# caizexin/GenVC

Hardware: AMD Instinct MI355X
Metric: utterances/s (streaming, 1 s chunks; with RTF and first-chunk latency) (higher is better)
Workload: dtype f32; 1 GPU; GenVC_small streaming, 1 s chunks, top_k=1, batch 1 per GPU (BASELINE configs[1]); parallelism=replicas x1, utterances sharded by rank, all_gather of token ids

## Files before the change

### genvc_amd/csrc/gemm.h

```cpp
#pragma once
#include "common.h"

namespace gvc {

__host__ __device__ __forceinline__ size_t fm16_index(int m, int k, int K) {
    return ((size_t)(m >> 4) * (K >> 4) + (k >> 4)) * 256 + (size_t)((((m & 15) + 16 * ((k & 15) >> 2)) << 2) + (k & 3));
}

enum GemmAct { ACT_NONE = 0, ACT_GELU_NEW = 1, ACT_RELU = 2, ACT_GELU_ERF = 3 };
enum GemmAAct { AACT_NONE = 0, AACT_LRELU = 1 };

struct GemmEpi {
    const float* bias;
    long long bias_batch_stride;
    int act;
    const float* resid;
    int ldr;
    long long resid_batch_stride;
    long long resid_batch_stride2;
    int resid_fm16;
    int geglu;
    const float* resid2;
    float out_scale;
    int c_fm16;
// ... 159 lines not shown
        } else {
            const int b = m / e.T, t = m - b * e.T;
            const int h = c / e.head_dim, j = c - h * e.head_dim;
            float* cache = which == 1 ? e.kcache : e.vcache;
            const size_t at = (((size_t)p.slot * e.n_head + h) * e.max_seq + (t + p.base)) * e.head_dim + j;
            if (e.kv_bf16) {
                ushort4 o;
                o.x = f32_to_bf16(v.x); o.y = f32_to_bf16(v.y); o.z = f32_to_bf16(v.z); o.w = f32_to_bf16(v.w);
                *reinterpret_cast<ushort4*>(reinterpret_cast<unsigned short*>(cache) + at) = o;
            } else {
                *reinterpret_cast<float4*>(cache + at) = v;
            }
        }
        return;
    }
    if (e.geglu) {
        *reinterpret_cast<float2*>(G.C + fm16_index(m, n >> 1, G.N >> 1)) = make_float2(gelu_erf(v.y) * v.x, gelu_erf(v.w) * v.z);
        return;
    }
    if (e.resid) {
        const float4 r = *reinterpret_cast<const float4*>(e.resid + (e.resid_fm16 ? fm16_index(m, n, G.N) : (size_t)m * e.ldr + n));
        v.x += r.x; v.y += r.y; v.z += r.z; v.w += r.w;
    }
    if (e.resid2) {
        const float4 r = *reinterpret_cast<const float4*>(e.resid2 + (size_t)m * e.ldr + n);
        v.x += r.x; v.y += r.y; v.z += r.z; v.w += r.w;
    }
    if (e.out_scale != 0.f) { v.x *= e.out_scale; v.y *= e.out_scale; v.z *= e.out_scale; v.w *= e.out_scale; }
    if (e.c_fm16) { *reinterpret_cast<float4*>(G.C + fm16_index(m, n, G.N)) = v; return; }
    *reinterpret_cast<float4*>(G.C + (size_t)m * G.ldc + n) = v;
}

typedef float f32x16 __attribute__((ext_vector_type(16)));

__global__ __launch_bounds__(256) void k_gemm_f32(const GemmArgs G);
__global__ void k_splitk_epilogue(const GemmArgs G);

int launch_gemm_skinny(GemmArgs G, int SK, long long work_cap, hipStream_t s);
int launch_ln_sum_rows(const float* x_in, float* x_out, float* a, const float* part, int SK, const float* bias, int rows, int d,
                       const float* ln_w, const float* ln_b, int a_fm16, hipStream_t s);
struct LnFuse {
    const float* x_in; float* x_out;
    const float* part; int SK; const float* pbias;
    const float* ln_w; const float* ln_b;
    int rows;
};
int launch_gemm_skinny_ln(GemmArgs G, const LnFuse& P, hipStream_t s);
int launch_gemm_strip(GemmArgs G, int sk_max, long long work_cap, int raw_partials, int* sk_used, hipStream_t s);
void gemm_init_attributes();
__global__ void k_to_fm16(const float* src, float* dst, int N, int K);
__global__ void k_to_fm16_bf16(const float* src, unsigned short* dst, int N, int K);

int launch_gemm_cap(GemmArgs G, int batch, long long work_cap, hipStream_t s);

}
```

### genvc_amd/csrc/gemm.hip

```cpp
#include "gemm.h"
#include "gemm_b16.h"
#include <algorithm>

namespace gvc {

constexpr int BM = 64, BN = 64, BK = 32, LDL = 36;

__global__ __launch_bounds__(256) void k_gemm_f32(const GemmArgs G) {
    __shared__ __attribute__((aligned(16))) float As[2][BM * LDL];
    __shared__ __attribute__((aligned(16))) float Bs[2][BN * LDL];
    const int tid = threadIdx.x, lane = tid & 63, wave = tid >> 6;
    const int wm = wave >> 1, wn = wave & 1;
    const int batch = blockIdx.z / G.SK, sk = blockIdx.z - batch * G.SK;
    const int m0 = blockIdx.y * BM, n0 = blockIdx.x * BN;
    const int ntile_all = (G.K + BK - 1) / BK;
    const int tps = (ntile_all + G.SK - 1) / G.SK;
    const int kbeg = sk * tps * BK;
    const int kend = min(G.K, kbeg + tps * BK);
    const int nt = kend > kbeg ? (kend - kbeg + BK - 1) / BK : 0;
    const float* Ab = G.A + gemm_boff(G, batch, G.a_batch_stride, G.a_batch_stride2);
    const float* Wb = G.Wt + gemm_binner(G, batch) * G.w_batch_stride;

    float4 ra[2], rb[2];
    auto load_tile = [&](int kt) {
// ... 34 lines not shown
    if (nt > 0) {
        load_tile(0);
        store_tile(0);
    }
    __syncthreads();
    int buf = 0;
    const int arow = (wm * 32 + (lane & 31)) * LDL + (lane >> 5) * 4;
    const int brow = (wn * 32 + (lane & 31)) * LDL + (lane >> 5) * 4;
    for (int kt = 0; kt < nt; ++kt) {
        if (kt + 1 < nt) load_tile(kt + 1);
#pragma unroll
        for (int kk = 0; kk < 4; ++kk) {
            const float4 a4 = *reinterpret_cast<const float4*>(&As[buf][arow + kk * 8]);
            const float4 b4 = *reinterpret_cast<const float4*>(&Bs[buf][brow + kk * 8]);
            acc = __builtin_amdgcn_mfma_f32_32x32x2f32(a4.x, b4.x, acc, 0, 0, 0);
            acc = __builtin_amdgcn_mfma_f32_32x32x2f32(a4.y, b4.y, acc, 0, 0, 0);
            acc = __builtin_amdgcn_mfma_f32_32x32x2f32(a4.z, b4.z, acc, 0, 0, 0);
            acc = __builtin_amdgcn_mfma_f32_32x32x2f32(a4.w, b4.w, acc, 0, 0, 0);
        }
        if (kt + 1 < nt) store_tile(buf ^ 1);
        __syncthreads();
        buf ^= 1;
    }

    const int n = n0 + wn * 32 + (lane & 31);
#pragma unroll
    for (int r = 0; r < 16; ++r) {
        const int m = m0 + wm * 32 + (r & 3) + 8 * (r >> 2) + 4 * (lane >> 5);
        if (m < G.M && n < G.N) {
            if (G.SK > 1)
                G.work[(((size_t)batch * G.SK + sk) * G.M + m) * G.N + n] = acc[r];
            else
                gemm_store(G, batch, m, n, acc[r]);
        }
    }
}

__global__ void k_splitk_epilogue(const GemmArgs G) {
    const int batch = blockIdx.z;
    const size_t mn = (size_t)G.M * G.N;
    for (size_t i = (size_t)blockIdx.x * blockDim.x + threadIdx.x; i < mn; i += (size_t)gridDim.x * blockDim.x) {
        const float* w = G.work + (size_t)batch * G.SK * mn + i;
        float pv[16];
#pragma unroll
        for (int s = 0; s < 16; ++s) pv[s] = w[(size_t)min(s, G.SK - 1) * mn];
        float v = 0.f;
#pragma unroll
        for (int s = 0; s < 16; ++s)
            if (s < G.SK) v += pv[s];
        gemm_store(G, batch, (int)(i / G.N), (int)(i % G.N), v);
    }
}

int launch_gemm_cap(GemmArgs G, int batch, long long work_cap, hipStream_t s) {
    GVC_REQUIRE(G.K % 4 == 0 && G.lda % 4 == 0 && G.ldw % 4 == 0 && G.conv_cin % 4 == 0 && G.conv_tap_stride % 4 == 0,
                GVC_ERR_ARG, "gemm: K/lda/ldw/conv strides must be multiples of 4 (K=%d lda=%d ldw=%d)", G.K, G.lda, G.ldw);
    const int tm = cdiv(G.M, BM), tn = cdiv(G.N, BN);
    const long long tiles = (long long)tm * tn * batch;
    int SK = 1;
    constexpr int sk_tiles = 128, sk_target = 192;
    if (tiles < sk_tiles && G.work) {
        SK = (int)((sk_target + tiles - 1) / tiles);
        const int max_by_k = G.K / (4 * BK) > 0 ? G.K / (4 * BK) : 1;
        if (SK > max_by_k) SK = max_by_k;
        if (SK > 16) SK = 16;
        while (SK > 1 && (long long)batch * SK * G.M * G.N > work_cap) --SK;
    } else if (tiles < 2 * sk_tiles && G.K >= 64 * BK && G.work) {
        SK = (int)((4 * sk_tiles + tiles - 1) / tiles);
        if (SK > G.K / (16 * BK)) SK = G.K / (16 * BK);
        while (SK > 1 && (long long)batch * SK * G.M * G.N > work_cap) --SK;
    }
    G.SK = SK;
    dim3 grid(tn, tm, batch * SK);
    hipLaunchKernelGGL(k_gemm_f32, grid, dim3(256), 0, s, G);
    GVC_LAUNCH_CHECK();
    if (SK > 1) {
        const long long mn = (long long)G.M * G.N;
        int gx = (int)((mn + 255) / 256);
        if (gx > 2048) gx = 2048;
        hipLaunchKernelGGL(k_splitk_epilogue, dim3(gx, 1, batch), dim3(256), 0, s, G);
        GVC_LAUNCH_CHECK();
    }
    return GVC_OK;
}

typedef float f32x4 __attribute__((ext_vector_type(4)));

template <int WB> struct WRaw { typedef float4 T; };
template <> struct WRaw<1> { typedef uint2 T; };
__device__ __forceinline__ float4 w_f4(const float4& r) { return r; }
__device__ __forceinline__ float4 w_f4(const uint2& u) {
    return make_float4(__uint_as_float(u.x << 16), __uint_as_float(u.x & 0xffff0000u), __uint_as_float(u.y << 16),
                       __uint_as_float(u.y & 0xffff0000u));
}

template <int MT, int NW, int WB = 0, int NC = 0>
__global__ __launch_bounds__(NW * 64) void k_gemm_skinny(const GemmArgs G) {
    extern __shared__ __attribute__((aligned(16))) float red_raw[];
    float (*red)[MT][256] = reinterpret_cast<float (*)[MT][256]>(red_raw);
    const int tid = threadIdx.x, lane = tid & 63, wave = tid >> 6;
    const int r = lane & 15, g = lane >> 4;
    const int n0 = blockIdx.x * 16;
    const int kslice = G.K / G.SK;
    const int kw = kslice / NW;
    const int kb16 = (blockIdx.y * kslice + wave * kw) >> 4;
    const int K16 = G.K >> 4;
    typedef typename WRaw<WB>::T wraw_t;
    const wraw_t* wp = reinterpret_cast<const wraw_t*>(G.Wt) + ((size_t)(n0 >> 4) * K16 + kb16) * 64 + lane;
    const float* ap[MT];
#pragma unroll
    for (int t = 0; t < MT; ++t) ap[t] = G.A + ((size_t)t * K16 + kb16) * 256 + lane * 4;
    f32x4 acc[MT];
#pragma unroll
    for (int t = 0; t < MT; ++t) acc[t] = {0.f, 0.f, 0.f, 0.f};
    EpiPre pre;
    {
        int pm, pn;
        bool four = false;
        if constexpr (MT <= 2) {
            pm = 16 * (tid >> 8) + 4 * (lane >> 4) + ((tid >> 6) & 3); pn = n0 + (lane & 15);
        } else {
            const bool pfm = G.SK == 1 && G.e.c_fm16;
            const int pt = tid >> 6, pj = tid & 63;
            pm = 16 * pt + (pfm ? (pj & 15) : (pj >> 2)); pn = n0 + 4 * (pfm ? (pj >> 4) : (pj & 3));
            four = true;
        }
        if (G.SK == 1) pre = gemm_prefetch(G, min(pm, G.M - 1), pn, four);
    }
    constexpr int U = NC > 0 ? (32 / (MT * NC) >= 8 ? 8 : 32 / (MT * NC)) : (32 / (1 + MT) >= 8 ? 8 : (32 / (1 + MT) >= 4 ? 4 : 2));
    float wn[MT][NC > 0 ? NC : 1], mc[MT][NC > 0 ? NC : 1], lc[MT][NC > 0 ? NC : 1];
    const float* pp[MT];
    if constexpr (NC > 0) {
        const int kg = blockIdx.y * kslice + wave * kw;
        const int h = kg / G.att_hd, pstride = G.att_hd + 4;
#pragma unroll
// ... 739 lines not shown
```

### genvc_amd/csrc/hubert.hip

```cpp
#include <map>
#include <string>
#include <vector>

#include "conv_lds.h"
#include "attn64.h"
#include <algorithm>

namespace gvc {

constexpr int kC0Chunk = 32;

static __global__ void k_hb_repack_conv(const float* w, float* out, int Co, int Ci, int k) {
    const size_t n = (size_t)Co * Ci * k;
    for (size_t i = (size_t)blockIdx.x * blockDim.x + threadIdx.x; i < n; i += (size_t)gridDim.x * blockDim.x) {
        const int j = (int)(i % k);
        const int ci = (int)((i / k) % Ci);
        const int co = (int)(i / ((size_t)k * Ci));
        out[((size_t)co * k + j) * Ci + ci] = w[i];
    }
}

static __global__ __launch_bounds__(256) void k_hb_conv0(const float* wav, const float* w, float* y, float* part, int T,
                                                        int T0, int C, int k, int stride) {
    extern __shared__ float xs[];
    const int b = blockIdx.z, chunk = blockIdx.x, tid = threadIdx.x;
    const int t0 = chunk * kC0Chunk;
    const int nt = min(kC0Chunk, T0 - t0);
    const int nx = (nt - 1) * stride + k;
    const float* src = wav + (size_t)b * T + (size_t)t0 * stride;
    for (int i = tid; i < nx; i += 256) xs[i] = src[i];
    __syncthreads();
    for (int c = blockIdx.y * 256 + tid; c < min(C, (int)(blockIdx.y + 1) * 256); c += 256) {
        float wr[16];
#pragma unroll
        for (int j = 0; j < 16; ++j) wr[j] = j < k ? w[(size_t)c * k + j] : 0.f;
        float s = 0.f, ss = 0.f, a = 0.f;
        float* yo = y + ((size_t)b * T0 + t0) * C + c;
        for (int t = 0; t < nt; ++t) {
            float acc = 0.f;
#pragma unroll
            for (int j = 0; j < 16; ++j)
                if (j < k) acc = fmaf(wr[j], xs[t * stride + j], acc);
            yo[(size_t)t * C] = acc;
            if (t == 0) a = acc;
            const float dv = acc - a;
            s += dv; ss = fmaf(dv, dv, ss);
        }
        float* po = part + (((size_t)b * gridDim.x + chunk) * C + c) * 2;
        const float dm = s / (float)nt;
        po[0] = a + dm; po[1] = fmaxf(ss - s * dm, 0.f);
    }
}

static __global__ __launch_bounds__(256) void k_hb_gn_stats(const float* part, float* stats, int nchunk, int T0, int C) {
    const int b = blockIdx.y, c = blockIdx.x * 8 + (threadIdx.x >> 5), l = threadIdx.x & 31;
    if (c >= C) return;
    double s = 0.0, ss = 0.0;
    for (int i0 = l; i0 < nchunk; i0 += 32 * 8) {
        float2 pv[8];
#pragma unroll
        for (int u = 0; u < 8; ++u)
            pv[u] = *reinterpret_cast<const float2*>(part + (((size_t)b * nchunk + min(i0 + 32 * u, nchunk - 1)) * C + c) * 2);
#pragma unroll
        for (int u = 0; u < 8; ++u)
            if (i0 + 32 * u < nchunk) {
                const double n = (double)min(kC0Chunk, T0 - (i0 + 32 * u) * kC0Chunk), m = (double)pv[u].x;
                s += n * m; ss += (double)pv[u].y + n * m * m;
            }
    }
#pragma unroll
    for (int o = 16; o >= 1; o >>= 1) { s += __shfl_xor(s, o, 32); ss += __shfl_xor(ss, o, 32); }
    if (l) return;
    const double mean = s / T0;
    double var = ss / T0 - mean * mean;
    if (var < 0.0) var = 0.0;
    stats[((size_t)b * C + c) * 2] = (float)mean;
    stats[((size_t)b * C + c) * 2 + 1] = (float)(1.0 / sqrt(var + 1e-5));
}
// ... 19 lines not shown
                                                          const float* part = nullptr, int SK = 0, const float* pbias = nullptr,
                                                          int rows = 0, float* dst_fm16 = nullptr) {
    __shared__ float red[4];
    const int row = blockIdx.x, tid = threadIdx.x;
    const int bi = row / rpb, ri = row - bi * rpb;
    const float* xr = src + bi * src_bs + (size_t)ri * d;
    float* orow = dst + bi * dst_bs + (size_t)ri * d;
    float4 v[4];
    float s = 0.f;
#pragma unroll
    for (int i = 0; i < 4; ++i) {
        const int k = (i * 256 + tid) * 4;
        v[i] = k < d ? *reinterpret_cast<const float4*>(xr + k) : make_float4(0.f, 0.f, 0.f, 0.f);
        if (part && k < d) {
            const float4 b4 = *reinterpret_cast<const float4*>(pbias + k);
            float4 p4[8];
#pragma unroll
            for (int sidx = 0; sidx < 8; ++sidx)
                p4[sidx] = *reinterpret_cast<const float4*>(part + ((size_t)min(sidx, SK - 1) * rows + row) * d + k);
            v[i].x += b4.x; v[i].y += b4.y; v[i].z += b4.z; v[i].w += b4.w;
#pragma unroll
            for (int sidx = 0; sidx < 8; ++sidx)
                if (sidx < SK) { v[i].x += p4[sidx].x; v[i].y += p4[sidx].y; v[i].z += p4[sidx].z; v[i].w += p4[sidx].w; }
        }
        s += (v[i].x + v[i].y) + (v[i].z + v[i].w);
    }
    const float inv_d = 1.0f / (float)d;
    const float mean = block4_sum(s, red) * inv_d;
    float q = 0.f;
#pragma unroll
    for (int i = 0; i < 4; ++i) {
        const int k = (i * 256 + tid) * 4;
        if (k < d) {
            const float a0 = v[i].x - mean, a1 = v[i].y - mean, a2 = v[i].z - mean, a3 = v[i].w - mean;
            q += (a0 * a0 + a1 * a1) + (a2 * a2 + a3 * a3);
        }
    }
    const float rstd = 1.0f / sqrtf(block4_sum(q, red) * inv_d + 1e-5f);
#pragma unroll
    for (int i = 0; i < 4; ++i) {
        const int k = (i * 256 + tid) * 4;
        if (k < d) {
            const float4 gw = *reinterpret_cast<const float4*>(w + k);
            const float4 gb = *reinterpret_cast<const float4*>(b + k);
            float4 o;
            o.x = (v[i].x - mean) * rstd * gw.x + gb.x; o.y = (v[i].y - mean) * rstd * gw.y + gb.y;
            o.z = (v[i].z - mean) * rstd * gw.z + gb.z; o.w = (v[i].w - mean) * rstd * gw.w + gb.w;
            *reinterpret_cast<float4*>(orow + k) = o;
            if (dst_fm16) *reinterpret_cast<float4*>(dst_fm16 + fm16_index(row, k, d)) = o;
        }
    }
}

static __global__ void k_hb_zero_pad(float* buf, int C, int T, int front, int back, const int32_t* fmask) {
    const int b = blockIdx.y;
    float* base = buf + (size_t)b * (front + T + back) * C;
    const size_t nf = (size_t)front * C, nb = (size_t)back * C;
    for (size_t i = (size_t)blockIdx.x * blockDim.x + threadIdx.x; i < nf + nb; i += (size_t)gridDim.x * blockDim.x) {
        if (i < nf) base[i] = 0.f;
        else base[(size_t)(front + T) * C + (i - nf)] = 0.f;
    }
    for (int t = blockIdx.x; t < T; t += gridDim.x) {
        if (!fmask[b * T + t]) continue;
        for (int i = threadIdx.x; i < C; i += blockDim.x) base[(size_t)(front + t) * C + i] = 0.f;
    }
}

static __global__ __launch_bounds__(64) void k_hb_frame_mask(const float* wav, int32_t* fmask, int T, int F) {
    const int f = blockIdx.x, b = blockIdx.y, lane = threadIdx.x;
    const int chunk = T / F;
    const float* p = wav + (size_t)b * T + (size_t)f * chunk;
    int nz = 0;
    for (int i = lane; i < chunk; i += 64) nz |= (p[i] != 0.f);
    nz = __any(nz);
    if (lane == 0) fmask[b * F + f] = nz ? 0 : 1;
}

}

using namespace gvc;

struct HbLin { float* w = nullptr; float* b = nullptr; int N = 0, K = 0; float* wf = nullptr;  };
struct HbLn { float* w = nullptr; float* b = nullptr; };
struct HbLayer { HbLin qkv, out, fc1, fc2; HbLn ln1, ln2; };

struct gvc_hubert {
    gvc_hubert_dims dm;
    int cg = 0, pad_front = 0, pad_back = 0;
    float* conv0_w = nullptr;
    HbLn gn;
    std::vector<float*> conv_w;
    std::vector<float*> conv_wp;
    int conv_lds = 1;
    int conv_lds_rows = 256;
    HbLn feat_ln, enc_ln;
    HbLin proj, pos, fin;
    std::vector<HbLayer> layers;
    std::map<std::string, int> bound;
    int n_expected = 0;
    float *act[2] = {nullptr, nullptr};
    float *part = nullptr, *stats = nullptr;
    int32_t* fmask = nullptr;
    float *xp = nullptr, *x = nullptr, *qkv = nullptr, *att = nullptr, *hbuf = nullptr, *tmp = nullptr, *work = nullptr;
    long long work_cap = 0;
    int max_frames = 0, max_t0 = 0;
    std::map<long long, hipGraphExec_t> graphs;
    hipStream_t cap_stream = nullptr;
    int use_graph = 1;
    int skinny = 1;
    int strip = 1;
    bool fm_ready = false;
    float *xf = nullptr, *af = nullptr, *hf = nullptr;
    std::vector<void*> allocs;
};

static int hb_alloc(gvc_hubert* c, float** p, size_t n) {
    GVC_CHECK_HIP(hipMalloc((void**)p, n * sizeof(float)));
    c->allocs.push_back(*p);
    return GVC_OK;
}
static int hb_alloc_lin(gvc_hubert* c, HbLin& L, int N, int K) {
    L.N = N; L.K = K;
    int rc = hb_alloc(c, &L.w, (size_t)N * K);
    return rc ? rc : hb_alloc(c, &L.b, N);
}
static int hb_alloc_ln(gvc_hubert* c, HbLn& L, int d) {
    int rc = hb_alloc(c, &L.w, d);
    return rc ? rc : hb_alloc(c, &L.b, d);
// ... 17 lines not shown
    const gvc_hubert_dims& D = *dims;
    GVC_REQUIRE(D.n_conv >= 2 && D.n_conv <= 8 && D.conv_kernel[0] <= 16, GVC_ERR_UNSUPPORTED, "hubert: need 2..8 conv layers, k0 <= 16");
    for (int i = 0; i < D.n_conv; ++i)
        GVC_REQUIRE(D.conv_dim[i] % 4 == 0 && D.conv_dim[i] <= 4096 && D.conv_kernel[i] >= 1 && D.conv_stride[i] >= 1,
                    GVC_ERR_UNSUPPORTED, "hubert: conv layer %d unsupported", i);
    GVC_REQUIRE(D.n_heads >= 1 && D.embed_dim == D.n_heads * 64, GVC_ERR_UNSUPPORTED, "hubert: head_dim must be 64");
    GVC_REQUIRE(D.embed_dim <= 4096 && D.ffn_dim % 4 == 0 && D.final_dim % 4 == 0 && D.pos_conv_groups >= 1 &&
                    D.embed_dim % D.pos_conv_groups == 0 && (D.embed_dim / D.pos_conv_groups) % 4 == 0 && D.pos_conv_kernel >= 1,
                GVC_ERR_UNSUPPORTED, "hubert: unsupported encoder dims");
    GVC_REQUIRE(D.max_batch >= 1 && hb_frames(D, D.max_samples, D.n_conv) >= 1, GVC_ERR_ARG, "hubert: bad capacity");
    auto* c = new gvc_hubert();
    c->dm = D;
    const int E = D.embed_dim, kp = D.pos_conv_kernel;
    c->cg = E / D.pos_conv_groups;
    c->pad_front = kp / 2;
    c->pad_back = kp - 1 - kp / 2;
    c->max_t0 = hb_frames(D, D.max_samples, 1);
    c->max_frames = hb_frames(D, D.max_samples, D.n_conv);
    int rc = hb_alloc(c, &c->conv0_w, (size_t)D.conv_dim[0] * D.conv_kernel[0]);
    if (!rc) rc = hb_alloc_ln(c, c->gn, D.conv_dim[0]);
    size_t maxact = 0;
    for (int i = 0, n = D.max_samples; i < D.n_conv; ++i) {
        n = (n - D.conv_kernel[i]) / D.conv_stride[i] + 1;
        maxact = std::max(maxact, (size_t)n * D.conv_dim[i]);
        if (i >= 1 && !rc) {
            float* w = nullptr;
            rc = hb_alloc(c, &w, (size_t)D.conv_dim[i] * D.conv_kernel[i] * D.conv_dim[i - 1]);
            c->conv_w.push_back(w);
            float* wp = nullptr;
            if (!rc && conv_lds_ci_ok(D.conv_dim[i - 1]) && D.conv_dim[i] % 16 == 0 &&
                conv_lds_bytes(D.conv_dim[i - 1], D.conv_kernel[i], 1, false, D.conv_stride[i]) <= kConvLdsMax)
                rc = hb_alloc(c, &wp, (size_t)D.conv_dim[i] * D.conv_kernel[i] * D.conv_dim[i - 1]);
            c->conv_wp.push_back(wp);
        }
    }
    const int Cl = D.conv_dim[D.n_conv - 1];
    if (!rc) rc = hb_alloc_ln(c, c->feat_ln, Cl);
    if (!rc) rc = hb_alloc_lin(c, c->proj, E, Cl);
    if (!rc) rc = hb_alloc_lin(c, c->pos, E, kp * c->cg);
    if (!rc) rc = hb_alloc_ln(c, c->enc_ln, E);
    c->layers.resize(D.n_layers);
    for (int l = 0; l < D.n_layers && !rc; ++l) {
        HbLayer& L = c->layers[l];
        if ((rc = hb_alloc_lin(c, L.qkv, 3 * E, E))) break;
        if ((rc = hb_alloc_lin(c, L.out, E, E))) break;
        if ((rc = hb_alloc_lin(c, L.fc1, D.ffn_dim, E))) break;
        if ((rc = hb_alloc_lin(c, L.fc2, E, D.ffn_dim))) break;
        if ((rc = hb_alloc_ln(c, L.ln1, E))) break;
        if ((rc = hb_alloc_ln(c, L.ln2, E))) break;
        for (HbLin* q : {&L.qkv, &L.out, &L.fc1, &L.fc2})
            if ((rc = hb_alloc(c, &q->wf, (size_t)q->N * q->K))) break;
    }
    if (!rc) rc = hb_alloc_lin(c, c->fin, D.final_dim, E);
    c->n_expected = 3 + (D.n_conv - 1) + 2 + 2 + 2 + 2 + 16 * D.n_layers + 2;
    const size_t B = D.max_batch, F = c->max_frames;
    for (int i = 0; i < 2 && !rc; ++i) rc = hb_alloc(c, &c->act[i], B * maxact);
    if (!rc) rc = hb_alloc(c, &c->part, B * (size_t)cdiv(c->max_t0, kC0Chunk) * D.conv_dim[0] * 2);
    if (!rc) rc = hb_alloc(c, &c->stats, B * D.conv_dim[0] * 2);
    if (!rc) rc = hb_alloc(c, reinterpret_cast<float**>(&c->fmask), B * F);
    if (!rc) rc = hb_alloc(c, &c->xp, B * (F + kp) * E);
    if (!rc) rc = hb_alloc(c, &c->x, B * F * E);
    if (!rc) rc = hb_alloc(c, &c->tmp, B * F * E);
    if (!rc) rc = hb_alloc(c, &c->att, B * F * E);
    if (!rc) rc = hb_alloc(c, &c->qkv, B * F * 3 * E);
    if (!rc) rc = hb_alloc(c, &c->hbuf, B * F * D.ffn_dim);
    const size_t fm_rows = std::max<size_t>(128, (B * F + 15) & ~(size_t)15);
    if (!rc) rc = hb_alloc(c, &c->xf, fm_rows * E);
    if (!rc) rc = hb_alloc(c, &c->af, fm_rows * E);
    if (!rc) rc = hb_alloc(c, &c->hf, fm_rows * D.ffn_dim);
    c->work_cap = 16ll << 20;
    if (!rc) rc = hb_alloc(c, &c->work, (size_t)c->work_cap);
    if (!rc && hipStreamCreateWithFlags(&c->cap_stream, hipStreamNonBlocking) != hipSuccess) rc = GVC_ERR_HIP;
    if (getenv("GVC_GRAPHS")) c->use_graph = atoi(getenv("GVC_GRAPHS"));
    conv_lds_init_attributes();
    if (E % 128 != 0 || D.ffn_dim % 128 != 0) c->skinny = 0;
    if (rc) { gvc_hubert_destroy(c); return rc; }
    *out = c;
    return GVC_OK;
}

extern "C" int gvc_hubert_destroy(gvc_hubert* c) {
    if (!c) return GVC_OK;
    for (auto& kv : c->graphs) hipGraphExecDestroy(kv.second);
    if (c->cap_stream) hipStreamDestroy(c->cap_stream);
    for (void* p : c->allocs) hipFree(p);
    delete c;
    return GVC_OK;
}

static int hb_copy(float* dst, const float* src, int64_t numel, int64_t expect, const char* name, hipStream_t s) {
    GVC_REQUIRE(numel == expect, GVC_ERR_ARG, "%s: expected %lld elements, got %lld", name, (long long)expect, (long long)numel);
    GVC_CHECK_HIP(hipMemcpyAsync(dst, src, numel * sizeof(float), hipMemcpyDeviceToDevice, s));
    return GVC_OK;
}

static bool ends_with(const std::string& n, const char* suf) {
    const size_t k = strlen(suf);
    return n.size() >= k && n.compare(n.size() - k, k, suf) == 0;
}

extern "C" int gvc_hubert_bind_weight(gvc_hubert* c, const char* name, const float* src, int64_t numel, gvc_stream sv) {
    GVC_REQUIRE(c && name && src, GVC_ERR_ARG, "gvc_hubert_bind_weight: null argument");
    hipStream_t s = (hipStream_t)sv;
    const gvc_hubert_dims& D = c->dm;
    const int E = D.embed_dim;
    std::string n(name);
// ... 49 lines not shown
    if (rc == GVC_OK && known) { c->bound[n] = 1; c->fm_ready = false; }
    return rc;
}

extern "C" int gvc_hubert_missing_weights(gvc_hubert* c) { return c ? c->n_expected - (int)c->bound.size() : -1; }

static int hb_linear(gvc_hubert* c, const HbLin& L, const float* A, float* C, int M, int act, const float* resid, hipStream_t s) {
    GemmArgs G;
    memset(&G, 0, sizeof(G));
    G.A = A; G.lda = L.K; G.Wt = L.w; G.ldw = L.K; G.C = C; G.ldc = L.N;
    G.M = M; G.N = L.N; G.K = L.K; G.work = c->work;
    G.e.bias = L.b; G.e.act = act;
    if (resid) { G.e.resid = resid; G.e.ldr = L.N; }
    return launch_gemm_cap(G, 1, c->work_cap, s);
}

static int hb_body(gvc_hubert* c, int B, int T, hipStream_t s) {
    const gvc_hubert_dims& D = c->dm;
    const int E = D.embed_dim;
    int rc;
    int Tin = hb_frames(D, T, 1);
    const int C0 = D.conv_dim[0];
    const int nchunk = cdiv(Tin, kC0Chunk);
    hipLaunchKernelGGL(k_hb_gn_stats, dim3(cdiv(C0, 8), B), dim3(256), 0, s, c->part, c->stats, nchunk, Tin, C0);
    GVC_LAUNCH_CHECK();
    {
        const size_t n4 = (size_t)Tin * C0 / 4;
        const int gx = (int)std::min<size_t>((n4 + 255) / 256, 4096);
        hipLaunchKernelGGL(k_hb_gn_gelu, dim3(gx, B), dim3(256), 0, s, c->act[0], c->stats, c->gn.w, c->gn.b, Tin, C0);
        GVC_LAUNCH_CHECK();
    }
    int cur = 0;
    for (int i = 1; i < D.n_conv; ++i) {
        const int Ci = D.conv_dim[i - 1], Co = D.conv_dim[i], k = D.conv_kernel[i], st = D.conv_stride[i];
        const int Tout = (Tin - k) / st + 1;
        if (c->conv_lds && c->conv_wp[i - 1] && Tout <= c->conv_lds_rows) {
            ConvLdsArgs A;
            memset(&A, 0, sizeof(A));
            A.x = c->act[cur]; A.x_bs = (long long)Tin * Ci; A.ldx = Ci; A.x_scale = 1.f; A.slope = 1.f;
            A.x_rows = Tin; A.stride = st;
            A.y = c->act[cur ^ 1]; A.y_bs = (long long)Tout * Co; A.ldy = Co;
            A.T = Tout; A.ntiles = Co / 16; A.act = ACT_GELU_ERF;
            A.job[0].wp = reinterpret_cast<const float4*>(c->conv_wp[i - 1]); A.job[0].k = k; A.job[0].dil = 1;
            if ((rc = launch_conv_lds(Ci, 1, A, 1, B, conv_lds_bytes(Ci, k, 1, false, st), s))) return rc;
            cur ^= 1;
            Tin = Tout;
            continue;
        }
        GemmArgs G;
        memset(&G, 0, sizeof(G));
        G.A = c->act[cur]; G.lda = st * Ci; G.a_batch_stride = (long long)Tin * Ci;
        G.Wt = c->conv_w[i - 1]; G.ldw = k * Ci;
        G.C = c->act[cur ^ 1]; G.ldc = Co; G.c_batch_stride = (long long)Tout * Co;
        G.M = Tout; G.N = Co; G.K = k * Ci; G.work = c->work;
        G.e.act = ACT_GELU_ERF;
        if ((rc = launch_gemm_cap(G, B, c->work_cap, s))) return rc;
        cur ^= 1;
        Tin = Tout;
    }
    const int F = Tin, Cl = D.conv_dim[D.n_conv - 1], rows = B * F;
    const int kp = D.pos_conv_kernel;
    const long long xp_bs = (long long)(F + kp - 1) * E;
    hipLaunchKernelGGL(k_hb_ln_rows, dim3(rows), dim3(256), 0, s, c->act[cur], (long long)F * Cl, c->act[cur ^ 1],
                       (long long)F * Cl, F, Cl, c->feat_ln.w, c->feat_ln.b);
    GVC_LAUNCH_CHECK();
    {
        GemmArgs G;
        memset(&G, 0, sizeof(G));
        G.A = c->act[cur ^ 1]; G.lda = Cl; G.a_batch_stride = (long long)F * Cl;
        G.Wt = c->proj.w; G.ldw = Cl;
        G.C = c->xp + (size_t)c->pad_front * E; G.ldc = E; G.c_batch_stride = xp_bs;
        G.M = F; G.N = E; G.K = Cl; G.work = c->work;
        G.e.bias = c->proj.b;
        if ((rc = launch_gemm_cap(G, B, c->work_cap, s))) return rc;
    }
    hipLaunchKernelGGL(k_hb_zero_pad, dim3(64, B), dim3(256), 0, s, c->xp, E, F, c->pad_front, c->pad_back, c->fmask);
    GVC_LAUNCH_CHECK();
    {
        GemmArgs G;
        memset(&G, 0, sizeof(G));
        const int cg = c->cg;
        G.batch_inner = D.pos_conv_groups;
        G.A = c->xp; G.lda = E; G.a_batch_stride = cg; G.a_batch_stride2 = xp_bs;
        G.conv_cin = cg; G.conv_tap_stride = E;
        G.Wt = c->pos.w; G.ldw = kp * cg; G.w_batch_stride = (long long)cg * kp * cg;
        G.C = c->tmp; G.ldc = E; G.c_batch_stride = cg; G.c_batch_stride2 = (long long)F * E;
        G.M = F; G.N = cg; G.K = kp * cg; G.work = c->work;
        G.e.bias = c->pos.b; G.e.bias_batch_stride = cg; G.e.act = ACT_GELU_ERF;
        G.e.resid = c->xp + (size_t)c->pad_front * E; G.e.ldr = E; G.e.resid_batch_stride = cg; G.e.resid_batch_stride2 = xp_bs;
        if ((rc = launch_gemm_cap(G, B * D.pos_conv_groups, c->work_cap, s))) return rc;
    }
    const bool skinny = c->skinny && (rows <= 128 || (c->strip && E % 64 == 0 && D.ffn_dim % 64 == 0));
    const bool strip = rows > 128;
    if (skinny) {
        hipLaunchKernelGGL(k_hb_ln_rows, dim3(rows), dim3(256), 0, s, c->tmp, (long long)F * E, c->x, (long long)F * E, F, E,
                           c->enc_ln.w, c->enc_ln.b, (const float*)nullptr, 0, (const float*)nullptr, rows, c->xf);
        GVC_LAUNCH_CHECK();
        int sk_used = 1;
        auto sk_gemm = [&](const HbLin& L, const float* A_fm, float* C, int act, int c_fm16, int SK, const float* resid = nullptr) {
            GemmArgs G;
            memset(&G, 0, sizeof(G));
            G.A = A_fm; G.lda = L.K; G.Wt = L.wf; G.ldw = L.K; G.C = C; G.ldc = L.N; G.M = rows; G.N = L.N; G.K = L.K;
            G.work = c->work;
            if (strip && resid) {
                if ((long long)rows * L.N > c->work_cap) { set_error("hubert: %d rows exceed the split-K work buffer", rows); return (int)GVC_ERR_ARG; }
                return launch_gemm_strip(G, 8, c->work_cap, 1, &sk_used, s);
            }
            sk_used = SK;
            if (SK == 1) { G.e.bias = L.b; G.e.act = act; G.e.c_fm16 = c_fm16; G.e.resid = resid; G.e.ldr = L.N; }
            if (strip) return launch_gemm_strip(G, 1, c->work_cap, 0, nullptr, s);
            return launch_gemm_skinny(G, SK, c->work_cap, s);
        };
        auto post_ln = [&](const HbLin& L, const HbLn& N, int) {
            const int SK = sk_used;
            if (SK > 1 || strip)
                hipLaunchKernelGGL(k_hb_ln_rows, dim3(rows), dim3(256), 0, s, c->x, (long long)F * E, c->x, (long long)F * E, F, E,
                                   N.w, N.b, c->work, SK, L.b, rows, c->xf);
            else
                hipLaunchKernelGGL(k_hb_ln_rows, dim3(rows), dim3(256), 0, s, c->tmp, (long long)F * E, c->x, (long long)F * E, F, E,
                                   N.w, N.b, (const float*)nullptr, 0, (const float*)nullptr, rows, c->xf);
        };
        const int sk_out = (E / 2) % 128 == 0 ? 2 : 1, sk_fc2 = (D.ffn_dim / 4) % 128 == 0 ? 4 : ((D.ffn_dim / 2) % 128 == 0 ? 2 : 1);
        for (int l = 0; l < D.n_layers; ++l) {
            const HbLayer& L = c->layers[l];
            if ((rc = sk_gemm(L.qkv, c->xf, c->qkv, ACT_NONE, 0, 1))) return rc;
            hipLaunchKernelGGL(k_attn64_mfma<true>, dim3(cdiv(F, 16), D.n_heads, B), dim3(256), 0, s, c->qkv, c->qkv + E, c->qkv + 2 * E, (long long)3 * E, (long long)F * 3 * E, F, F, c->af, F, E, 0.125f, 1, c->fmask);
            GVC_LAUNCH_CHECK();
            if ((rc = sk_gemm(L.out, c->af, c->tmp, ACT_NONE, 0, sk_out, c->x))) return rc;
            post_ln(L.out, L.ln1, sk_out);
            GVC_LAUNCH_CHECK();
            if ((rc = sk_gemm(L.fc1, c->xf, c->hf, ACT_GELU_ERF, 1, 1))) return rc;
            if ((rc = sk_gemm(L.fc2, c->hf, c->tmp, ACT_NONE, 0, sk_fc2, c->x))) return rc;
            post_ln(L.fc2, L.ln2, sk_fc2);
            GVC_LAUNCH_CHECK();
        }
        return GVC_OK;
    }
    hipLaunchKernelGGL(k_hb_ln_rows, dim3(rows), dim3(256), 0, s, c->tmp, (long long)F * E, c->x, (long long)F * E, F, E,
                       c->enc_ln.w, c->enc_ln.b);
    GVC_LAUNCH_CHECK();
    for (int l = 0; l < D.n_layers; ++l) {
        const HbLayer& L = c->layers[l];
        if ((rc = hb_linear(c, L.qkv, c->x, c->qkv, rows, ACT_NONE, nullptr, s))) return rc;
        hipLaunchKernelGGL(k_attn64_mfma<true>, dim3(cdiv(F, 16), D.n_heads, B), dim3(256), 0, s, c->qkv, c->qkv + E, c->qkv + 2 * E, (long long)3 * E, (long long)F * 3 * E, F, F, c->att, F, E, 0.125f, 0, c->fmask);
        GVC_LAUNCH_CHECK();
        if ((rc = hb_linear(c, L.out, c->att, c->tmp, rows, ACT_NONE, c->x, s))) return rc;
        hipLaunchKernelGGL(k_hb_ln_rows, dim3(rows), dim3(256), 0, s, c->tmp, (long long)F * E, c->x, (long long)F * E, F, E,
                           L.ln1.w, L.ln1.b);
        GVC_LAUNCH_CHECK();
        if ((rc = hb_linear(c, L.fc1, c->x, c->hbuf, rows, ACT_GELU_ERF, nullptr, s))) return rc;
        if ((rc = hb_linear(c, L.fc2, c->hbuf, c->tmp, rows, ACT_NONE, c->x, s))) return rc;
        hipLaunchKernelGGL(k_hb_ln_rows, dim3(rows), dim3(256), 0, s, c->tmp, (long long)F * E, c->x, (long long)F * E, F, E,
                           L.ln2.w, L.ln2.b);
        GVC_LAUNCH_CHECK();
    }
    return GVC_OK;
}

extern "C" int gvc_hubert_forward(gvc_hubert* c, const float* wav, int32_t B, int32_t T, float* out, gvc_stream sv) {
    GVC_REQUIRE(c && wav && out, GVC_ERR_ARG, "gvc_hubert_forward: null argument");
    GVC_REQUIRE(gvc_hubert_missing_weights(c) == 0, GVC_ERR_STATE, "%d HuBERT weight tensors are not bound",
                gvc_hubert_missing_weights(c));
    const gvc_hubert_dims& D = c->dm;
    const int F = hb_frames(D, T, D.n_conv);
    GVC_REQUIRE(B >= 1 && B <= D.max_batch && T <= D.max_samples && F >= 1, GVC_ERR_ARG,
                "hubert: B=%d samples=%d outside capacity (%d, %d) or too short", B, T, D.max_batch, D.max_samples);
    hipStream_t s = (hipStream_t)sv;
    if (c->skinny && !c->fm_ready) {
        for (HbLayer& L : c->layers)
            for (HbLin* q : {&L.qkv, &L.out, &L.fc1, &L.fc2}) {
                hipLaunchKernelGGL(k_to_fm16, dim3(1024), dim3(256), 0, s, q->w, q->wf, q->N, q->K);
                GVC_LAUNCH_CHECK();
            }
        c->fm_ready = true;
    }
    const int T0 = hb_frames(D, T, 1), C0 = D.conv_dim[0], k0 = D.conv_kernel[0], s0 = D.conv_stride[0];
    hipLaunchKernelGGL(k_hb_conv0, dim3(cdiv(T0, kC0Chunk), cdiv(C0, 256), B), dim3(256), ((kC0Chunk - 1) * s0 + k0) * sizeof(float), s, wav,
                       c->conv0_w, c->act[0], c->part, T, T0, C0, k0, s0);
    GVC_LAUNCH_CHECK();
    hipLaunchKernelGGL(k_hb_frame_mask, dim3(F, B), dim3(64), 0, s, wav, c->fmask, T, F);
    GVC_LAUNCH_CHECK();
    int rc;
    if (!c->use_graph) {
        if ((rc = hb_body(c, B, T, s))) return rc;
    } else {
        const long long key = ((long long)B << 32) | (unsigned)T;
        auto it = c->graphs.find(key);
        if (it == c->graphs.end()) {
            if (c->graphs.size() >= 64) {
                for (auto& kv : c->graphs) hipGraphExecDestroy(kv.second);
                c->graphs.clear();
            }
            hipGraphExec_t ge;
            if ((rc = capture_graph(c->cap_stream, &ge, [&] { return hb_body(c, B, T, c->cap_stream); }))) return rc;
            it = c->graphs.emplace(key, ge).first;
        }
        GVC_CHECK_HIP(hipGraphLaunch(it->second, s));
    }
    {
        GemmArgs G;
        memset(&G, 0, sizeof(G));
        const HbLin& L = c->fin;
        G.A = c->x; G.lda = L.K; G.Wt = L.w; G.ldw = L.K; G.C = out; G.ldc = L.N;
        G.M = B * F; G.N = L.N; G.K = L.K; G.work = c->work;
        G.e.bias = L.b;
        if ((rc = launch_gemm_cap(G, 1, c->work_cap, s))) return rc;
    }
    return GVC_OK;
}
```

Measured before the change: 7.074 utterances/s.

## Fuse HuBERT front-end kernels and route small GEMMs to skinny/row-tiled paths

Several fusions go into the HuBERT front end. The frame-mask computation moves into the conv0 kernel. The projection split-K reduction and bias are folded into the zero-pad kernel. The positional-conv split-K reduction, GELU, residual and encoder LayerNorm become one kernel. Conv feature-extractor GEMMs use a new MFMA row-tiled kernel with a register prefetch pipeline and intra-block K split instead of split-K plus an epilogue. The projection and final GEMMs use the skinny fm16 path for small row counts. The aim is fewer launches and less round-trip of partials through global memory, at the cost of more code paths and extra fm16 weight copies.

```diff
diff --git a/genvc_amd/csrc/gemm.h b/genvc_amd/csrc/gemm.h
--- a/genvc_amd/csrc/gemm.h
+++ b/genvc_amd/csrc/gemm.h
@@ -235,5 +235,7 @@
 __global__ void k_to_fm16_bf16(const float* src, unsigned short* dst, int N, int K);
 
 int launch_gemm_cap(GemmArgs G, int batch, long long work_cap, hipStream_t s);
-
-}
+int launch_gemm_cap_raw(GemmArgs G, int batch, long long work_cap, int* sk_used, hipStream_t s);
+int launch_gemm_rows(GemmArgs G, int batch, hipStream_t s);
+
+}
diff --git a/genvc_amd/csrc/gemm.hip b/genvc_amd/csrc/gemm.hip
--- a/genvc_amd/csrc/gemm.hip
+++ b/genvc_amd/csrc/gemm.hip
@@ -110,7 +110,7 @@
     }
 }
 
-int launch_gemm_cap(GemmArgs G, int batch, long long work_cap, hipStream_t s) {
+static int gemm_cap_impl(GemmArgs G, int batch, long long work_cap, int* sk_raw, hipStream_t s) {
     GVC_REQUIRE(G.K % 4 == 0 && G.lda % 4 == 0 && G.ldw % 4 == 0 && G.conv_cin % 4 == 0 && G.conv_tap_stride % 4 == 0,
                 GVC_ERR_ARG, "gemm: K/lda/ldw/conv strides must be multiples of 4 (K=%d lda=%d ldw=%d)", G.K, G.lda, G.ldw);
     const int tm = cdiv(G.M, BM), tn = cdiv(G.N, BN);
@@ -132,6 +132,7 @@
     dim3 grid(tn, tm, batch * SK);
     hipLaunchKernelGGL(k_gemm_f32, grid, dim3(256), 0, s, G);
     GVC_LAUNCH_CHECK();
+    if (sk_raw) { *sk_raw = SK; return GVC_OK; }
     if (SK > 1) {
         const long long mn = (long long)G.M * G.N;
         int gx = (int)((mn + 255) / 256);
@@ -139,6 +140,153 @@
         hipLaunchKernelGGL(k_splitk_epilogue, dim3(gx, 1, batch), dim3(256), 0, s, G);
         GVC_LAUNCH_CHECK();
     }
+    return GVC_OK;
+}
+
+int launch_gemm_cap(GemmArgs G, int batch, long long work_cap, hipStream_t s) { return gemm_cap_impl(G, batch, work_cap, nullptr, s); }
+int launch_gemm_cap_raw(GemmArgs G, int batch, long long work_cap, int* sk_used, hipStream_t s) { return gemm_cap_impl(G, batch, work_cap, sk_used, s); }
+
+template <int WM, int WN, int WK>
+__global__ __launch_bounds__(256) void k_gemm_f32_t(const GemmArgs G) {
+    static_assert(WM * WN * WK == 4 && 4 % WK == 0, "four waves");
+    constexpr int TM = 32 * WM, TN = 32 * WN, KS = 4 / WK, NP = WM * WN, PF = 3;
+    constexpr int kTile = (TM + TN) * LDL;
+    static_assert(2 * kTile >= 4 * 1024, "the accumulator exchange reuses the staging buffers");
+    __shared__ __attribute__((aligned(16))) float sm[2 * kTile];
+    const int tid = threadIdx.x, lane = tid & 63, wave = tid >> 6;
+    const int wk = wave / NP, wm = (wave % NP) / WN, wn = wave % WN;
+    const int batch = blockIdx.z;
+    const int m0 = blockIdx.y * TM, n0 = blockIdx.x * TN;
+    const int nt = (G.K + BK - 1) / BK;
+    const float* Ab = G.A + gemm_boff(G, batch, G.a_batch_stride, G.a_batch_stride2);
+    const float* Wb = G.Wt + gemm_binner(G, batch) * G.w_batch_stride;
+    typedef float v4f __attribute__((ext_vector_type(4)));
+    struct Regs { v4f a[WM], b[WN]; };
+    constexpr int NL = WM + WN;
+    const int lr = tid >> 3, lc4 = (tid & 7) * 4;
+    const int rot = (3 * blockIdx.y + 7 * (blockIdx.x >> 3)) % max(nt, 1);
+    auto tile_k = [&](int kt) __attribute__((always_inline)) { return (kt + rot < nt ? kt + rot : kt + rot - nt) * BK + lc4; };
+    const float* ap[WM];
+    const float* bp[WN];
+#pragma unroll
+    for (int j = 0; j < WM; ++j) ap[j] = Ab + (size_t)min(m0 + lr + 32 * j, G.M - 1) * G.lda;
+#pragma unroll
+    for (int j = 0; j < WN; ++j) bp[j] = Wb + (size_t)min(n0 + lr + 32 * j, G.N - 1) * G.ldw;
+    auto load_tile = [&](int kt, Regs& R) __attribute__((always_inline)) {
+        const int k = min(tile_k(min(kt, nt - 1)), G.K - 4);
+#pragma unroll
+        for (int j = 0; j < WM; ++j) asm volatile("global_load_dwordx4 %0, %1, off" : "=v"(R.a[j]) : "v"(ap[j] + k) : "memory");
+#pragma unroll
+        for (int j = 0; j < WN; ++j) asm volatile("global_load_dwordx4 %0, %1, off" : "=v"(R.b[j]) : "v"(bp[j] + k) : "memory");
+    };
+    auto await_tile = [&](Regs& R) __attribute__((always_inline)) {
+        asm volatile("s_waitcnt vmcnt(%0)" ::"n"(2 * NL) : "memory");
+#pragma unroll
+        for (int j = 0; j < WM; ++j) asm volatile("" : "+v"(R.a[j]));
+#pragma unroll
+        for (int j = 0; j < WN; ++j) asm volatile("" : "+v"(R.b[j]));
+    };
+    auto store_tile = [&](int buf, int kt, Regs& R) __attribute__((always_inline)) {
+        await_tile(R);
+        float* As = sm + buf * kTile;
+        float* Bs = As + TM * LDL;
+        const bool live = tile_k(kt) < G.K;
+        const v4f z = {0.f, 0.f, 0.f, 0.f};
+#pragma unroll
+        for (int j = 0; j < WM; ++j) {
+            v4f v = R.a[j];
+            if (!live) v = z;
+            *reinterpret_cast<v4f*>(&As[(lr + 32 * j) * LDL + lc4]) = v;
+        }
+#pragma unroll
+        for (int j = 0; j < WN; ++j) {
+            v4f v = R.b[j];
+            if (!live) v = z;
+            *reinterpret_cast<v4f*>(&Bs[(lr + 32 * j) * LDL + lc4]) = v;
+        }
+    };
+    f32x16 acc;
+#pragma unroll
+    for (int i = 0; i < 16; ++i) acc[i] = 0.f;
+    const int arow = (wm * 32 + (lane & 31)) * LDL + (lane >> 5) * 4 + wk * KS * 8;
+    const int brow = TM * LDL + (wn * 32 + (lane & 31)) * LDL + (lane >> 5) * 4 + wk * KS * 8;
+    auto multiply = [&](int buf) __attribute__((always_inline)) {
+        const float* T = sm + buf * kTile;
+#pragma unroll
+        for (int kk = 0; kk < KS; ++kk) {
+            const float4 a4 = *reinterpret_cast<const float4*>(&T[arow + kk * 8]);
+            const float4 b4 = *reinterpret_cast<const float4*>(&T[brow + kk * 8]);
+            acc = __builtin_amdgcn_mfma_f32_32x32x2f32(a4.x, b4.x, acc, 0, 0, 0);
+            acc = __builtin_amdgcn_mfma_f32_32x32x2f32(a4.y, b4.y, acc, 0, 0, 0);
+            acc = __builtin_amdgcn_mfma_f32_32x32x2f32(a4.z, b4.z, acc, 0, 0, 0);
+            acc = __builtin_amdgcn_mfma_f32_32x32x2f32(a4.w, b4.w, acc, 0, 0, 0);
+        }
+    };
+    Regs r0, r1, r2;
+    load_tile(0, r0);
+    load_tile(1, r1);
+    load_tile(2, r2);
+    store_tile(0, 0, r0);
+    __syncthreads();
+    auto retire = [&](Regs& R) __attribute__((always_inline)) {
+#pragma unroll
+        for (int j = 0; j < WM; ++j) asm volatile("" : "+v"(R.a[j]));
+#pragma unroll
+        for (int j = 0; j < WN; ++j) asm volatile("" : "+v"(R.b[j]));
+    };
+    auto step = [&](int kt, Regs& freed, Regs& next) __attribute__((always_inline)) {
+        load_tile(kt + PF, freed);
+        multiply(kt & 1);
+        store_tile((kt + 1) & 1, min(kt + 1, nt - 1), next);
+        if (kt + 1 >= nt) {
+            asm volatile("s_waitcnt vmcnt(0)" ::: "memory");
+            retire(r0);
+            retire(r1);
+            retire(r2);
+        }
+        __syncthreads();
+    };
+    for (int kt = 0; kt < nt; kt += PF) {
+        step(kt, r0, r1);
+        if (kt + 1 >= nt) break;
+        step(kt + 1, r1, r2);
+        if (kt + 2 >= nt) break;
+        step(kt + 2, r2, r0);
+    }
+    if constexpr (WK == 1) {
+        const int n = n0 + wn * 32 + (lane & 31);
+#pragma unroll
+        for (int r = 0; r < 16; ++r) {
+            const int m = m0 + wm * 32 + (r & 3) + 8 * (r >> 2) + 4 * (lane >> 5);
+            if (m < G.M && n < G.N) gemm_store(G, batch, m, n, acc[r]);
+        }
+    } else {
+#pragma unroll
+        for (int r = 0; r < 16; ++r) sm[wave * 1024 + r * 64 + lane] = acc[r];
+        __syncthreads();
+        for (int e = tid; e < NP * 1024; e += 256) {
+            const int p = e >> 10, idx = e & 1023, r = idx >> 6, ln = idx & 63;
+            float v = 0.f;
+#pragma unroll
+            for (int w = 0; w < WK; ++w) v += sm[(w * NP + p) * 1024 + idx];
+            const int m = m0 + (p / WN) * 32 + (r & 3) + 8 * (r >> 2) + 4 * (ln >> 5);
+            const int n = n0 + (p % WN) * 32 + (ln & 31);
+            if (m < G.M && n < G.N) gemm_store(G, batch, m, n, v);
+        }
+    }
+}
+
+constexpr long long kRowsFill = 192;
+int launch_gemm_rows(GemmArgs G, int batch, hipStream_t s) {
+    GVC_REQUIRE(G.M >= 1 && G.N >= 1 && G.K >= 4 && G.K % 4 == 0 && G.lda % 4 == 0 && G.ldw % 4 == 0 && G.conv_cin == 0 && G.a_act == 0 && !G.e.qkv && !G.e.c_fm16, GVC_ERR_ARG,
+                "gemm rows: unsupported operands (K=%d lda=%d ldw=%d)", G.K, G.lda, G.ldw);
+    G.SK = 1;
+    const long long t64 = (long long)cdiv(G.M, 64) * cdiv(G.N, 64) * batch, t32 = (long long)cdiv(G.M, 32) * cdiv(G.N, 64) * batch;
+    auto grid = [&](int tm, int tn) { return dim3(cdiv(G.N, tn), cdiv(G.M, tm), batch); };
+    if (t64 >= kRowsFill) hipLaunchKernelGGL((k_gemm_f32_t<2, 2, 1>), grid(64, 64), dim3(256), 0, s, G);
+    else if (t32 >= kRowsFill) hipLaunchKernelGGL((k_gemm_f32_t<1, 2, 2>), grid(32, 64), dim3(256), 0, s, G);
+    else hipLaunchKernelGGL((k_gemm_f32_t<1, 1, 4>), grid(32, 32), dim3(256), 0, s, G);
+    GVC_LAUNCH_CHECK();
     return GVC_OK;
 }
 
diff --git a/genvc_amd/csrc/hubert.hip b/genvc_amd/csrc/hubert.hip
--- a/genvc_amd/csrc/hubert.hip
+++ b/genvc_amd/csrc/hubert.hip
@@ -21,9 +21,19 @@
 }
 
 static __global__ __launch_bounds__(256) void k_hb_conv0(const float* wav, const float* w, float* y, float* part, int T,
-                                                        int T0, int C, int k, int stride) {
+                                                        int T0, int C, int k, int stride, int32_t* fmask, int F) {
     extern __shared__ float xs[];
     const int b = blockIdx.z, chunk = blockIdx.x, tid = threadIdx.x;
+    if (blockIdx.y == 0) {
+        const int per = T / F, lane = tid & 63;
+        for (int f = chunk * 4 + (tid >> 6); f < F; f += gridDim.x * 4) {
+            const float* p = wav + (size_t)b * T + (size_t)f * per;
+            int nz = 0;
+            for (int i = lane; i < per; i += 64) nz |= (p[i] != 0.f);
+            nz = __any(nz);
+            if (lane == 0) fmask[b * F + f] = nz ? 0 : 1;
+        }
+    }
     const int t0 = chunk * kC0Chunk;
     const int nt = min(kC0Chunk, T0 - t0);
     const int nx = (nt - 1) * stride + k;
@@ -149,7 +159,8 @@
     }
 }
 
-static __global__ void k_hb_zero_pad(float* buf, int C, int T, int front, int back, const int32_t* fmask) {
+static __global__ void k_hb_zero_pad(float* buf, int C, int T, int front, int back, const int32_t* fmask,
+                                     const float* part = nullptr, int SK = 0, const float* pbias = nullptr, int rows = 0) {
     const int b = blockIdx.y;
     float* base = buf + (size_t)b * (front + T + back) * C;
     const size_t nf = (size_t)front * C, nb = (size_t)back * C;
@@ -158,19 +169,85 @@
         else base[(size_t)(front + T) * C + (i - nf)] = 0.f;
     }
     for (int t = blockIdx.x; t < T; t += gridDim.x) {
-        if (!fmask[b * T + t]) continue;
-        for (int i = threadIdx.x; i < C; i += blockDim.x) base[(size_t)(front + t) * C + i] = 0.f;
-    }
-}
-
-static __global__ __launch_bounds__(64) void k_hb_frame_mask(const float* wav, int32_t* fmask, int T, int F) {
-    const int f = blockIdx.x, b = blockIdx.y, lane = threadIdx.x;
-    const int chunk = T / F;
-    const float* p = wav + (size_t)b * T + (size_t)f * chunk;
-    int nz = 0;
-    for (int i = lane; i < chunk; i += 64) nz |= (p[i] != 0.f);
-    nz = __any(nz);
-    if (lane == 0) fmask[b * F + f] = nz ? 0 : 1;
+        const bool pad = fmask[b * T + t] != 0;
+        float* row = base + (size_t)(front + t) * C;
+        if (pad) {
+            for (int i = threadIdx.x; i < C; i += blockDim.x) row[i] = 0.f;
+        } else if (part) {
+            for (int i = threadIdx.x * 4; i < C; i += blockDim.x * 4) {
+                float4 p4[8];
+#pragma unroll
+                for (int sidx = 0; sidx < 8; ++sidx)
+                    p4[sidx] = *reinterpret_cast<const float4*>(part + ((size_t)min(sidx, SK - 1) * rows + (size_t)b * T + t) * C + i);
+                const float4 b4 = *reinterpret_cast<const float4*>(pbias + i);
+                float4 v = make_float4(0.f, 0.f, 0.f, 0.f);
+#pragma unroll
+                for (int sidx = 0; sidx < 8; ++sidx)
+                    if (sidx < SK) { v.x += p4[sidx].x; v.y += p4[sidx].y; v.z += p4[sidx].z; v.w += p4[sidx].w; }
+                v.x += b4.x; v.y += b4.y; v.z += b4.z; v.w += b4.w;
+                *reinterpret_cast<float4*>(row + i) = v;
+            }
+        }
+    }
+}
+
+static __global__ __launch_bounds__(256) void k_hb_pos_ln(const float* xp, long long xp_bs, int front, const float* part, int SK, int groups,
+                                                         int cg, const float* pbias, float* dst, int F, int d, const float* w,
+                                                         const float* b, float* dst_fm16) {
+    __shared__ float red[4];
+    const int row = blockIdx.x, tid = threadIdx.x;
+    const int bi = row / F, t = row - bi * F;
+    const float* xr = xp + bi * xp_bs + (size_t)(front + t) * d;
+    float* orow = dst + (size_t)row * d;
+    float4 v[4];
+    float s = 0.f;
+#pragma unroll
+    for (int i = 0; i < 4; ++i) {
+        const int k = (i * 256 + tid) * 4;
+        v[i] = make_float4(0.f, 0.f, 0.f, 0.f);
+        if (k < d) {
+            const int g = k / cg, n = k - g * cg;
+            const float* pp = part + (((size_t)(bi * groups + g) * SK) * F + t) * cg + n;
+            const size_t ps = (size_t)F * cg;
+            const float4 x4 = *reinterpret_cast<const float4*>(xr + k);
+            const float4 b4 = *reinterpret_cast<const float4*>(pbias + k);
+            float4 p4[16];
+#pragma unroll
+            for (int sidx = 0; sidx < 16; ++sidx) p4[sidx] = *reinterpret_cast<const float4*>(pp + (size_t)min(sidx, SK - 1) * ps);
+            float4 a = make_float4(0.f, 0.f, 0.f, 0.f);
+#pragma unroll
+            for (int sidx = 0; sidx < 16; ++sidx)
+                if (sidx < SK) { a.x += p4[sidx].x; a.y += p4[sidx].y; a.z += p4[sidx].z; a.w += p4[sidx].w; }
+            v[i].x = gelu_erf(a.x + b4.x) + x4.x; v[i].y = gelu_erf(a.y + b4.y) + x4.y;
+            v[i].z = gelu_erf(a.z + b4.z) + x4.z; v[i].w = gelu_erf(a.w + b4.w) + x4.w;
+        }
+        s += (v[i].x + v[i].y) + (v[i].z + v[i].w);
+    }
+    const float inv_d = 1.0f / (float)d;
+    const float mean = block4_sum(s, red) * inv_d;
+    float q = 0.f;
+#pragma unroll
+    for (int i = 0; i < 4; ++i) {
+        const int k = (i * 256 + tid) * 4;
+        if (k < d) {
+            const float a0 = v[i].x - mean, a1 = v[i].y - mean, a2 = v[i].z - mean, a3 = v[i].w - mean;
+            q += (a0 * a0 + a1 * a1) + (a2 * a2 + a3 * a3);
+        }
+    }
+    const float rstd = 1.0f / sqrtf(block4_sum(q, red) * inv_d + 1e-5f);
+#pragma unroll
+    for (int i = 0; i < 4; ++i) {
+        const int k = (i * 256 + tid) * 4;
+        if (k < d) {
+            const float4 gw = *reinterpret_cast<const float4*>(w + k);
+            const float4 gb = *reinterpret_cast<const float4*>(b + k);
+            float4 o;
+            o.x = (v[i].x - mean) * rstd * gw.x + gb.x; o.y = (v[i].y - mean) * rstd * gw.y + gb.y;
+            o.z = (v[i].z - mean) * rstd * gw.z + gb.z; o.w = (v[i].w - mean) * rstd * gw.w + gb.w;
+            *reinterpret_cast<float4*>(orow + k) = o;
+            if (dst_fm16) *reinterpret_cast<float4*>(dst_fm16 + fm16_index(row, k, d)) = o;
+        }
+    }
 }
 
 }
@@ -294,6 +371,8 @@
             if ((rc = hb_alloc(c, &q->wf, (size_t)q->N * q->K))) break;
     }
     if (!rc) rc = hb_alloc_lin(c, c->fin, D.final_dim, E);
+    for (HbLin* q : {&c->proj, &c->fin})
+        if (!rc) rc = hb_alloc(c, &q->wf, (size_t)q->N * q->K);
     c->n_expected = 3 + (D.n_conv - 1) + 2 + 2 + 2 + 2 + 16 * D.n_layers + 2;
     const size_t B = D.max_batch, F = c->max_frames;
     for (int i = 0; i < 2 && !rc; ++i) rc = hb_alloc(c, &c->act[i], B * maxact);
@@ -449,19 +528,28 @@
         G.A = c->act[cur]; G.lda = st * Ci; G.a_batch_stride = (long long)Tin * Ci;
         G.Wt = c->conv_w[i - 1]; G.ldw = k * Ci;
         G.C = c->act[cur ^ 1]; G.ldc = Co; G.c_batch_stride = (long long)Tout * Co;
-        G.M = Tout; G.N = Co; G.K = k * Ci; G.work = c->work;
+        G.M = Tout; G.N = Co; G.K = k * Ci;
         G.e.act = ACT_GELU_ERF;
-        if ((rc = launch_gemm_cap(G, B, c->work_cap, s))) return rc;
+        if ((rc = launch_gemm_rows(G, B, s))) return rc;
         cur ^= 1;
         Tin = Tout;
     }
     const int F = Tin, Cl = D.conv_dim[D.n_conv - 1], rows = B * F;
     const int kp = D.pos_conv_kernel;
     const long long xp_bs = (long long)(F + kp - 1) * E;
+    const int proj_sk = (Cl / 2) % 128 == 0 ? 2 : 1;
+    const bool proj_skinny = c->skinny && rows <= 128 && Cl % 64 == 0 && Cl <= D.ffn_dim && (long long)proj_sk * rows * E <= c->work_cap;
     hipLaunchKernelGGL(k_hb_ln_rows, dim3(rows), dim3(256), 0, s, c->act[cur], (long long)F * Cl, c->act[cur ^ 1],
-                       (long long)F * Cl, F, Cl, c->feat_ln.w, c->feat_ln.b);
+                       (long long)F * Cl, F, Cl, c->feat_ln.w, c->feat_ln.b, (const float*)nullptr, 0, (const float*)nullptr, rows,
+                       proj_skinny ? c->hf : (float*)nullptr);
     GVC_LAUNCH_CHECK();
-    {
+    if (proj_skinny) {
+        GemmArgs G;
+        memset(&G, 0, sizeof(G));
+        G.A = c->hf; G.lda = Cl; G.Wt = c->proj.wf; G.ldw = Cl; G.C = c->work; G.ldc = E; G.M = rows; G.N = E; G.K = Cl;
+        G.work = c->work;
+        if ((rc = launch_gemm_skinny(G, proj_sk, c->work_cap, s))) return rc;
+    } else {
         GemmArgs G;
         memset(&G, 0, sizeof(G));
         G.A = c->act[cur ^ 1]; G.lda = Cl; G.a_batch_stride = (long long)F * Cl;
@@ -471,8 +559,13 @@
         G.e.bias = c->proj.b;
         if ((rc = launch_gemm_cap(G, B, c->work_cap, s))) return rc;
     }
-    hipLaunchKernelGGL(k_hb_zero_pad, dim3(64, B), dim3(256), 0, s, c->xp, E, F, c->pad_front, c->pad_back, c->fmask);
+    if (proj_skinny)
+        hipLaunchKernelGGL(k_hb_zero_pad, dim3(64, B), dim3(256), 0, s, c->xp, E, F, c->pad_front, c->pad_back, c->fmask,
+                           (const float*)c->work, proj_sk, (const float*)c->proj.b, rows);
+    else
+        hipLaunchKernelGGL(k_hb_zero_pad, dim3(64, B), dim3(256), 0, s, c->xp, E, F, c->pad_front, c->pad_back, c->fmask);
     GVC_LAUNCH_CHECK();
+    int pos_sk = 1;
     {
         GemmArgs G;
         memset(&G, 0, sizeof(G));
@@ -485,13 +578,20 @@
         G.M = F; G.N = cg; G.K = kp * cg; G.work = c->work;
         G.e.bias = c->pos.b; G.e.bias_batch_stride = cg; G.e.act = ACT_GELU_ERF;
         G.e.resid = c->xp + (size_t)c->pad_front * E; G.e.ldr = E; G.e.resid_batch_stride = cg; G.e.resid_batch_stride2 = xp_bs;
-        if ((rc = launch_gemm_cap(G, B * D.pos_conv_groups, c->work_cap, s))) return rc;
-    }
+        if ((rc = launch_gemm_cap_raw(G, B * D.pos_conv_groups, c->work_cap, &pos_sk, s))) return rc;
+    }
+    auto enc_ln = [&](float* fm) {
+        if (pos_sk > 1)
+            hipLaunchKernelGGL(k_hb_pos_ln, dim3(rows), dim3(256), 0, s, c->xp, xp_bs, c->pad_front, (const float*)c->work, pos_sk,
+                               D.pos_conv_groups, c->cg, (const float*)c->pos.b, c->x, F, E, c->enc_ln.w, c->enc_ln.b, fm);
+        else
+            hipLaunchKernelGGL(k_hb_ln_rows, dim3(rows), dim3(256), 0, s, c->tmp, (long long)F * E, c->x, (long long)F * E, F, E,
+                               c->enc_ln.w, c->enc_ln.b, (const float*)nullptr, 0, (const float*)nullptr, rows, fm);
+    };
     const bool skinny = c->skinny && (rows <= 128 || (c->strip && E % 64 == 0 && D.ffn_dim % 64 == 0));
     const bool strip = rows > 128;
     if (skinny) {
-        hipLaunchKernelGGL(k_hb_ln_rows, dim3(rows), dim3(256), 0, s, c->tmp, (long long)F * E, c->x, (long long)F * E, F, E,
-                           c->enc_ln.w, c->enc_ln.b, (const float*)nullptr, 0, (const float*)nullptr, rows, c->xf);
+        enc_ln(c->xf);
         GVC_LAUNCH_CHECK();
         int sk_used = 1;
         auto sk_gemm = [&](const HbLin& L, const float* A_fm, float* C, int act, int c_fm16, int SK, const float* resid = nullptr) {
@@ -533,8 +633,7 @@
         }
         return GVC_OK;
     }
-    hipLaunchKernelGGL(k_hb_ln_rows, dim3(rows), dim3(256), 0, s, c->tmp, (long long)F * E, c->x, (long long)F * E, F, E,
-                       c->enc_ln.w, c->enc_ln.b);
+    enc_ln(nullptr);
     GVC_LAUNCH_CHECK();
     for (int l = 0; l < D.n_layers; ++l) {
         const HbLayer& L = c->layers[l];
@@ -569,13 +668,16 @@
                 hipLaunchKernelGGL(k_to_fm16, dim3(1024), dim3(256), 0, s, q->w, q->wf, q->N, q->K);
                 GVC_LAUNCH_CHECK();
             }
+        for (HbLin* q : {&c->proj, &c->fin})
+            if (q->N % 16 == 0 && q->K % 16 == 0) {
+                hipLaunchKernelGGL(k_to_fm16, dim3(1024), dim3(256), 0, s, q->w, q->wf, q->N, q->K);
+                GVC_LAUNCH_CHECK();
+            }
         c->fm_ready = true;
     }
     const int T0 = hb_frames(D, T, 1), C0 = D.conv_dim[0], k0 = D.conv_kernel[0], s0 = D.conv_stride[0];
     hipLaunchKernelGGL(k_hb_conv0, dim3(cdiv(T0, kC0Chunk), cdiv(C0, 256), B), dim3(256), ((kC0Chunk - 1) * s0 + k0) * sizeof(float), s, wav,
-                       c->conv0_w, c->act[0], c->part, T, T0, C0, k0, s0);
-    GVC_LAUNCH_CHECK();
-    hipLaunchKernelGGL(k_hb_frame_mask, dim3(F, B), dim3(64), 0, s, wav, c->fmask, T, F);
+                       c->conv0_w, c->act[0], c->part, T, T0, C0, k0, s0, c->fmask, F);
     GVC_LAUNCH_CHECK();
     int rc;
     if (!c->use_graph) {
@@ -601,7 +703,10 @@
         G.A = c->x; G.lda = L.K; G.Wt = L.w; G.ldw = L.K; G.C = out; G.ldc = L.N;
         G.M = B * F; G.N = L.N; G.K = L.K; G.work = c->work;
         G.e.bias = L.b;
-        if ((rc = launch_gemm_cap(G, 1, c->work_cap, s))) return rc;
+        if (c->skinny && B * F <= 128 && L.N % 16 == 0 && L.K % 64 == 0) {
+            G.A = c->xf; G.Wt = L.wf;
+            if ((rc = launch_gemm_skinny(G, 1, c->work_cap, s))) return rc;
+        } else if ((rc = launch_gemm_cap(G, 1, c->work_cap, s))) return rc;
     }
     return GVC_OK;
 }
```

Result: no change. 7.069 utterances/s (-0.1%).
